# Zejun-Yang/AniPortrait

Measured on NVIDIA H100. Metric: denoised frames/sec @512x512 L=16 steps=25, higher is better.
Workload: dtype fp16

## Files before the change

### aniportrait_b200/csrc/ap_gemm.cu

```cuda
#include <stdio.h>
#include <stdlib.h>

#include "ap_host.h"
#include "ap_ptx.cuh"
#include "ap_wgmma.cuh"

namespace ap {

enum { A_GEMM = 0, A_CONV_S1 = 1, A_CONV_S2 = 2 };
enum { EPI_LINEAR = 0, EPI_GEGLU = 1 };

struct GemmParams {
  int M, N;
  int num_m_tiles, num_n_tiles, num_kb;
  int a_mode;
  int kb_src1, kb_src2;
  int Nf, Ho, Wo;
  int bw, bh, bn;
  int tiles_x, tiles_y;
  int C1, C2;
  const float* bias;
  int bias_group_rows;
  long long bias_ld;
  const __half* residual;
  int ldr;
  __half* out;
  int ldo;
  int out_al16, res_al16;
  int n_valid;
  int out_f32;
  int gelu;
  int quick_gelu;
  int tma_epi;
  int sub_w, sub_h, sub_n;
  int epi_double;
  int debug;
  float2* row_stat_out;
  long long row_stat_ld;
  float2* col_stat_out;
  long long col_stat_ld;
  const float* ln_rstd;
};


template <int BN, int EPI>
struct GemmCfg {
  static constexpr int BM = 128;
  static constexpr int BK = 64;
  static constexpr int A_BYTES = BM * BK * 2;
  static constexpr int B_BYTES = BN * BK * 2;
  static constexpr int STAGE_BYTES = A_BYTES + B_BYTES;
  static constexpr int EPI_STAGING = 8 * 4096;
  static constexpr int ACC_PW = EPI == EPI_GEGLU ? 128 : 64;
  static constexpr int ACC_LD = ACC_PW + 8;
  static constexpr int ACC_STAGING = 2 * 64 * ACC_LD * 4;
  static constexpr int MAX_SMEM = 227 * 1024 - 1024  - 256  - EPI_STAGING - ACC_STAGING;
  static constexpr int STAGES_RAW = MAX_SMEM / STAGE_BYTES;
  static constexpr int STAGES = STAGES_RAW > 8 ? 8 : STAGES_RAW;
  static constexpr int SMEM_BYTES = STAGES * STAGE_BYTES + EPI_STAGING + ACC_STAGING + 1024 + 256;
  static_assert(STAGES >= 2, "need at least a double-buffered operand ring");
  static_assert(B_BYTES % 1024 == 0, "B stage must keep 1024B alignment");
};


template <int BN, int EPI>
__global__ void __launch_bounds__(384, 1)
gemm_kernel(const __grid_constant__ CUtensorMap tmA1, const __grid_constant__ CUtensorMap tmA2,
            const __grid_constant__ CUtensorMap tmB, const __grid_constant__ CUtensorMap tmOut,
            const __grid_constant__ CUtensorMap tmRes, const GemmParams p) {
  using Cfg = GemmCfg<BN, EPI>;
  constexpr int STAGES = Cfg::STAGES;
  griddep_launch_dependents();
  extern __shared__ uint8_t smem_raw[];
  uint8_t* smem = reinterpret_cast<uint8_t*>((reinterpret_cast<uintptr_t>(smem_raw) + 1023) & ~uintptr_t(1023));
  uint8_t* smem_a = smem;
  uint8_t* smem_b = smem + STAGES * Cfg::A_BYTES;
  uint8_t* smem_epi = smem + STAGES * Cfg::STAGE_BYTES;
  float* smem_acc = reinterpret_cast<float*>(smem_epi + Cfg::EPI_STAGING);
  uint64_t* full_bar = reinterpret_cast<uint64_t*>(smem_acc + 2 * 64 * Cfg::ACC_LD);
  uint64_t* empty_bar = full_bar + STAGES;
  uint64_t* res_bar = empty_bar + STAGES;

  const int warp = threadIdx.x >> 5;
  const int lane = threadIdx.x & 31;
  const int n_groups = p.num_n_tiles;
  const int num_tiles = p.num_m_tiles * n_groups;
  const int first_tile = blockIdx.x;
  const int tile_stride = gridDim.x;

  if (warp == 0 && lane == 0) {
    tma_prefetch_desc(&tmA1);
    tma_prefetch_desc(&tmB);
    if (p.kb_src2 > 0) tma_prefetch_desc(&tmA2);
    for (int s = 0; s < STAGES; ++s) {
      mbar_init(&full_bar[s], 1);
      mbar_init(&empty_bar[s], 8);
    }
    for (int s = 0; s < 8; ++s) mbar_init(&res_bar[s], 1);
    if (p.tma_epi) {
      tma_prefetch_desc(&tmOut);
      if (p.residual != nullptr) tma_prefetch_desc(&tmRes);
    }
    fence_mbar_init();
  }
  __syncthreads();
  griddep_wait();

  if (warp < 4) {
    setmaxnreg_dec<40>();
    if (warp != 0) return;
    int stage = 0;
    uint32_t phase = 0;
    for (int tile = first_tile; tile < num_tiles; tile += tile_stride) {
      const int m_tile = tile / n_groups;
      const int n_tile = tile % n_groups;
      int n0 = 0, y0 = 0, x0 = 0;
      if (p.a_mode != A_GEMM) {
        const int per_frame = p.tiles_x * p.tiles_y;
        const int tn = m_tile / per_frame;
        const int rem = m_tile % per_frame;
        n0 = tn * p.bn;
        y0 = (rem / p.tiles_x) * p.bh;
        x0 = (rem % p.tiles_x) * p.bw;
      }
      int within = 0, kx = 0, ky = 0;
      for (int kb = 0; kb < p.num_kb; ++kb) {
        mbar_wait_quiet(&empty_bar[stage], phase ^ 1);
        if (elect_one()) {
          if (p.debug == 1) {
            mbar_arrive(&full_bar[stage]);
          } else {
            const bool load_a = !(p.debug == 4 && (kb & 1)), load_b = !(p.debug == 3 && (kb & 1));
            mbar_arrive_expect_tx(&full_bar[stage], (load_a ? Cfg::A_BYTES : 0) + (load_b ? Cfg::B_BYTES : 0));
            void* a_dst = smem_a + stage * Cfg::A_BYTES;
            void* b_dst = smem_b + stage * Cfg::B_BYTES;
            const bool second = within >= p.kb_src1;
            const CUtensorMap* am = second ? &tmA2 : &tmA1;
            const int c0 = (second ? within - p.kb_src1 : within) * Cfg::BK;
            if (!load_a) {
            } else if (p.a_mode == A_GEMM) {
              tma_load_2d(am, &full_bar[stage], a_dst, c0, m_tile * Cfg::BM);
            } else if (p.a_mode == A_CONV_S1) {
              tma_load_4d(am, &full_bar[stage], a_dst, c0, x0 + kx - 1, y0 + ky - 1, n0);
            } else {
              const int px = (kx == 1) ? 0 : 1, dx = (kx == 0) ? -1 : 0;
              const int py = (ky == 1) ? 0 : 1, dy = (ky == 0) ? -1 : 0;
              tma_load_5d(am, &full_bar[stage], a_dst, px * (second ? p.C2 : p.C1) + c0, x0 + dx, py, y0 + dy, n0);
            }
            if (load_b) tma_load_2d(&tmB, &full_bar[stage], b_dst, kb * Cfg::BK, n_tile * BN);
          }
        }
        __syncwarp();
        if (++within == p.kb_src1 + p.kb_src2) {
          within = 0;
          if (++kx == 3) { kx = 0; ++ky; }
        }
        if (++stage == STAGES) { stage = 0; phase ^= 1; }
      }
    }
    return;
  }

  setmaxnreg_inc<232>();
  const int wg = (warp >> 2) - 1;
  const int wq = warp & 3;
  const int lane_group = 2 * wg + (wq & 1);
  const int col_half = wq >> 1;
  const int row = lane_group * 32 + lane;
  const int r0 = lane_group * 32;
  float* acc_stage = smem_acc + wg * 64 * Cfg::ACC_LD;
  const float* acc_row = acc_stage + ((wq & 1) * 32 + lane) * Cfg::ACC_LD;
  constexpr int ACC_PER_CHUNK = (EPI == EPI_GEGLU) ? 64 : 32;
  constexpr int NCHUNK = BN / ACC_PER_CHUNK;
  constexpr int NPASS = (BN + Cfg::ACC_PW - 1) / Cfg::ACC_PW;
  const uint32_t a_base = smem_u32(smem_a) + wg * (64 * 128), b_base = smem_u32(smem_b);
  int stage = 0;
  uint32_t phase = 0;

  const int ew = warp - 4;
  uint8_t* obuf0 = smem_epi + ew * 4096;
  uint8_t* rbuf = obuf0 + 2048;
  uint32_t ochunk = 0;
  uint64_t* rbar = &res_bar[ew];
  uint32_t rphase = 0;
  const bool has_res = (EPI == EPI_LINEAR) && p.residual != nullptr;
  const int sw = (lane >> 1) & 3;
  float ln_next = 1.f;
  auto ln_prefetch = [&](int tile_) {
    if (tile_ >= num_tiles) return;
    const long long mm = (long long)(tile_ / n_groups) * Cfg::BM + r0 + lane;
    ln_next = mm < p.M ? __ldg(p.ln_rstd + mm) : 1.f;
  };
  if (p.tma_epi && p.ln_rstd != nullptr) ln_prefetch(first_tile);

  float acc[BN / 2];
  for (int tile = first_tile; tile < num_tiles; tile += tile_stride) {
    const int m_tile = tile / n_groups;
    const int n_tile = tile % n_groups;
    int prev_stage = -1;
    for (int kb = 0; kb < p.num_kb; ++kb) {
      mbar_wait_quiet(&full_bar[stage], phase);
      if (p.debug != 2) {
        wgmma_fence();
        const uint64_t da = wgmma_desc_k_sw128(a_base + stage * Cfg::A_BYTES);
        const uint64_t db = wgmma_desc_k_sw128(b_base + stage * Cfg::B_BYTES);
#pragma unroll
        for (int k = 0; k < Cfg::BK / 16; ++k) wgmma_ss<BN>(acc, da + 2 * k, db + 2 * k, (kb | k) != 0);
        wgmma_commit();
      }
      wgmma_wait<1>();
      if (prev_stage >= 0) {
        __syncwarp();
        if (lane == 0) mbar_arrive(&empty_bar[prev_stage]);
      }
      prev_stage = stage;
      if (++stage == STAGES) { stage = 0; phase ^= 1; }
    }
    wgmma_wait<0>();
    reg_fence<BN / 2>(acc);
    __syncwarp();
    if (lane == 0 && prev_stage >= 0) mbar_arrive(&empty_bar[prev_stage]);

    int cy = 0, cx = 0, cn = 0;
    long long m = 0;
    bool row_ok = true;
    if (p.a_mode == A_GEMM) {
      cy = m_tile * Cfg::BM + r0;
      m = (long long)cy + lane;
      row_ok = m < p.M;
    } else {
      const int per_frame = p.tiles_x * p.tiles_y;
      const int tn = m_tile / per_frame;
      const int rem = m_tile % per_frame;
      cn = tn * p.bn + r0 / (p.bh * p.bw);
      cy = (rem / p.tiles_x) * p.bh + (r0 / p.bw) % p.bh;
      cx = (rem % p.tiles_x) * p.bw + r0 % p.bw;
      const int n = tn * p.bn + row / (p.bh * p.bw);
      const int y = (rem / p.tiles_x) * p.bh + (row / p.bw) % p.bh;
      const int x = (rem % p.tiles_x) * p.bw + row % p.bw;
      row_ok = (n < p.Nf) && (y < p.Ho) && (x < p.Wo);
      m = ((long long)n * p.Ho + y) * p.Wo + x;
    }
    const float* bias_row = nullptr;
    if (p.bias != nullptr) bias_row = p.bias + (row_ok ? (m / p.bias_group_rows) : 0) * p.bias_ld;
    float ln_a = 1.f;
    if (p.tma_epi && p.ln_rstd != nullptr) {
      ln_a = ln_next;
      ln_prefetch(tile + tile_stride);
    }
    float rs_s = 0.f, rs_q = 0.f;
    const bool want_stats = (EPI == EPI_LINEAR) && (p.row_stat_out != nullptr || p.col_stat_out != nullptr);
    auto load_res = [&](int chunk) {
      if (lane == 0) {
        mbar_arrive_expect_tx(rbar, 2048);
        const int col = n_tile * BN + chunk * 32;
        if (p.a_mode == A_GEMM) tma_load_2d(&tmRes, rbar, rbuf, col, cy);
        else tma_load_4d(&tmRes, rbar, rbuf, col, cx, cy, cn);
      }
    };
    if (p.tma_epi && has_res && col_half < NCHUNK) load_res(col_half);

    auto chunk_tma = [&](int c, const float* src) {
      const int acol = n_tile * BN + c * ACC_PER_CHUNK;
      float v[32];
      if (EPI == EPI_GEGLU) {
#pragma unroll
        for (int h = 0; h < 2; ++h) {
          float bv[16], bg[16];
#pragma unroll
          for (int j = 0; j < 16; ++j) { bv[j] = 0.f; bg[j] = 0.f; }
          if (bias_row != nullptr) {
            const float4* b4 = reinterpret_cast<const float4*>(bias_row + acol + h * 32);
#pragma unroll
            for (int j = 0; j < 4; ++j) {
              const float4 a = __ldg(b4 + j), g = __ldg(b4 + 4 + j);
              bv[4 * j] = a.x; bv[4 * j + 1] = a.y; bv[4 * j + 2] = a.z; bv[4 * j + 3] = a.w;
              bg[4 * j] = g.x; bg[4 * j + 1] = g.y; bg[4 * j + 2] = g.z; bg[4 * j + 3] = g.w;
            }
          }
#pragma unroll
          for (int j = 0; j < 16; ++j)
            v[h * 16 + j] = fmaf(src[h * 32 + j], ln_a, bv[j]) * gelu_erf(fmaf(src[h * 32 + 16 + j], ln_a, bg[j]));
        }
      } else {
#pragma unroll
        for (int j = 0; j < 8; ++j) {
          const float4 a = reinterpret_cast<const float4*>(src)[j];
          v[4 * j] = a.x; v[4 * j + 1] = a.y; v[4 * j + 2] = a.z; v[4 * j + 3] = a.w;
        }
        if (p.ln_rstd != nullptr) {
          const float4* b4 = reinterpret_cast<const float4*>(bias_row + acol);
#pragma unroll
          for (int j = 0; j < 8; ++j) {
            const float4 b = __ldg(b4 + j);
            v[4 * j + 0] = fmaf(v[4 * j + 0], ln_a, b.x);
            v[4 * j + 1] = fmaf(v[4 * j + 1], ln_a, b.y);
            v[4 * j + 2] = fmaf(v[4 * j + 2], ln_a, b.z);
            v[4 * j + 3] = fmaf(v[4 * j + 3], ln_a, b.w);
          }
        } else if (bias_row != nullptr) {
          const float4* b4 = reinterpret_cast<const float4*>(bias_row + acol);
#pragma unroll
          for (int j = 0; j < 8; ++j) {
            const float4 b = __ldg(b4 + j);
            v[4 * j + 0] += b.x; v[4 * j + 1] += b.y; v[4 * j + 2] += b.z; v[4 * j + 3] += b.w;
          }
        }
        if (p.gelu) {
#pragma unroll
          for (int j = 0; j < 32; ++j) v[j] = gelu_erf(v[j]);
        } else if (p.quick_gelu) {
#pragma unroll
          for (int j = 0; j < 32; ++j) v[j] = quick_gelu(v[j]);
        }
        if (has_res) {
          mbar_wait_quiet(rbar, rphase);
          rphase ^= 1;
#pragma unroll
          for (int q = 0; q < 4; ++q) {
            const uint4 u = *reinterpret_cast<const uint4*>(rbuf + lane * 64 + ((q ^ sw) << 4));
            const __half2* h2 = reinterpret_cast<const __half2*>(&u);
#pragma unroll
            for (int j = 0; j < 4; ++j) {
              const float2 f = __half22float2(h2[j]);
              v[q * 8 + 2 * j] += f.x;
              v[q * 8 + 2 * j + 1] += f.y;
            }
          }
        }
      }
      const bool dbl = !has_res && p.epi_double;
      uint8_t* obuf = (dbl && (ochunk & 1)) ? rbuf : obuf0;
      ++ochunk;
      if (lane == 0) {
        if (dbl) tma_store_wait_read<1>();
        else tma_store_wait_read<0>();
      }
      __syncwarp();
      if (want_stats && !row_ok) {
#pragma unroll
        for (int j = 0; j < 32; ++j) v[j] = 0.f;
      }
#pragma unroll
      for (int q = 0; q < 4; ++q) {
        __half2 o[4];
#pragma unroll
        for (int j = 0; j < 4; ++j) o[j] = __floats2half2_rn(v[q * 8 + 2 * j], v[q * 8 + 2 * j + 1]);
        if (EPI == EPI_LINEAR && p.row_stat_out != nullptr) {
#pragma unroll
          for (int j = 0; j < 4; ++j) {
            const float2 f = __half22float2(o[j]);
            rs_s += f.x + f.y;
            rs_q = fmaf(f.x, f.x, fmaf(f.y, f.y, rs_q));
          }
        }
        *reinterpret_cast<uint4*>(obuf + lane * 64 + ((q ^ sw) << 4)) = *reinterpret_cast<uint4*>(o);
      }
      fence_proxy_async_smem();
      __syncwarp();
      if (EPI == EPI_LINEAR && p.col_stat_out != nullptr) {
        const int hc = lane & 15, rp = lane >> 4;
        float s0 = 0.f, s1 = 0.f, q0 = 0.f, q1 = 0.f;
#pragma unroll
        for (int rr = 0; rr < 16; ++rr) {
          const int rw = 2 * rr + rp;
          const uint32_t u = *reinterpret_cast<const uint32_t*>(
              obuf + rw * 64 + ((((hc >> 2) ^ ((rw >> 1) & 3))) << 4) + ((hc & 3) << 2));
          const float2 f = __half22float2(*reinterpret_cast<const __half2*>(&u));
          s0 += f.x; q0 = fmaf(f.x, f.x, q0);
          s1 += f.y; q1 = fmaf(f.y, f.y, q1);
        }
        s0 += __shfl_xor_sync(0xffffffffu, s0, 16);
        q0 += __shfl_xor_sync(0xffffffffu, q0, 16);
        s1 += __shfl_xor_sync(0xffffffffu, s1, 16);
        q1 += __shfl_xor_sync(0xffffffffu, q1, 16);
        if (lane < 16) {
          float4* dst = reinterpret_cast<float4*>(p.col_stat_out + (long long)(m_tile * 4 + lane_group) * p.col_stat_ld +
                                                  n_tile * BN + c * 32 + 2 * hc);
          *dst = make_float4(s0, q0, s1, q1);
        }
      }
      if (has_res && c + 2 < NCHUNK) load_res(c + 2);
      if (lane == 0) {
        const int ocol = n_tile * (BN / (EPI == EPI_GEGLU ? 2 : 1)) + c * 32;
        if (p.a_mode == A_GEMM) tma_store_2d(&tmOut, obuf, ocol, cy);
        else tma_store_4d(&tmOut, obuf, ocol, cx, cy, cn);
        tma_store_commit();
      }
    };

    auto chunk_direct = [&](int c, const float* src) {
      if (EPI == EPI_GEGLU) {
#pragma unroll
        for (int h = 0; h < 2; ++h) {
          const int ncol = n_tile * BN + c * 64 + h * 32;
          const float* s = src + h * 32;
          float v[32];
#pragma unroll
          for (int j = 0; j < 32; ++j) v[j] = s[j] + (bias_row != nullptr ? __ldg(bias_row + ncol + j) : 0.f);
          const int ocol = ncol >> 1;
          if (row_ok) {
            __half2 o[8];
#pragma unroll
            for (int j = 0; j < 8; ++j) {
              const float a0 = v[2 * j] * gelu_erf(v[16 + 2 * j]);
              const float a1 = v[2 * j + 1] * gelu_erf(v[16 + 2 * j + 1]);
              o[j] = __floats2half2_rn(a0, a1);
            }
            __half* dst = p.out + m * p.ldo + ocol;
            if (ocol + 16 <= p.n_valid && (p.ldo & 7) == 0 && p.out_al16) {
              uint4* d4 = reinterpret_cast<uint4*>(dst);
              d4[0] = *reinterpret_cast<uint4*>(&o[0]);
              d4[1] = *reinterpret_cast<uint4*>(&o[4]);
            } else {
              const __half* oh = reinterpret_cast<const __half*>(o);
              for (int j = 0; j < 16; ++j)
                if (ocol + j < p.n_valid) dst[j] = oh[j];
            }
          }
        }
        return;
      }
      const int ncol = n_tile * BN + c * 32;
      float v[32];
#pragma unroll
      for (int j = 0; j < 32; ++j) v[j] = src[j];
      if (bias_row != nullptr) {
        const float4* b4 = reinterpret_cast<const float4*>(bias_row + ncol);
#pragma unroll
        for (int j = 0; j < 8; ++j) {
          const float4 b = __ldg(b4 + j);
          v[4 * j + 0] += b.x; v[4 * j + 1] += b.y; v[4 * j + 2] += b.z; v[4 * j + 3] += b.w;
        }
      }
      if (p.gelu) {
#pragma unroll
        for (int j = 0; j < 32; ++j) v[j] = gelu_erf(v[j]);
      } else if (p.quick_gelu) {
#pragma unroll
        for (int j = 0; j < 32; ++j) v[j] = quick_gelu(v[j]);
      }
      if (!row_ok) return;
      const bool vec_ok = (ncol + 32 <= p.n_valid) && ((p.ldo & 7) == 0) && p.out_al16;
      if (p.residual != nullptr) {
        if (ncol + 32 <= p.n_valid && (p.ldr & 7) == 0 && p.res_al16) {
          const uint4* r4 = reinterpret_cast<const uint4*>(p.residual + m * p.ldr + ncol);
#pragma unroll
          for (int q = 0; q < 4; ++q) {
            const uint4 u = __ldg(r4 + q);
            const __half2* h2 = reinterpret_cast<const __half2*>(&u);
#pragma unroll
            for (int j = 0; j < 4; ++j) {
              const float2 f = __half22float2(h2[j]);
              v[q * 8 + 2 * j] += f.x;
              v[q * 8 + 2 * j + 1] += f.y;
            }
          }
        } else {
          const __half* rs = p.residual + m * p.ldr + ncol;
          for (int j = 0; j < 32; ++j)
            if (ncol + j < p.n_valid) v[j] += __half2float(rs[j]);
        }
      }
      __half* dst = p.out + m * p.ldo + ncol;
      if (p.out_f32) {
        float* dstf = reinterpret_cast<float*>(p.out) + m * p.ldo + ncol;
        for (int j = 0; j < 32; ++j)
          if (ncol + j < p.n_valid) dstf[j] = v[j];
      } else if (vec_ok) {
        uint4* d4 = reinterpret_cast<uint4*>(dst);
#pragma unroll
        for (int q = 0; q < 4; ++q) {
          __half2 o[4];
#pragma unroll
          for (int j = 0; j < 4; ++j) o[j] = __floats2half2_rn(v[q * 8 + 2 * j], v[q * 8 + 2 * j + 1]);
          d4[q] = *reinterpret_cast<uint4*>(o);
        }
      } else {
        for (int j = 0; j < 32; ++j)
          if (ncol + j < p.n_valid) dst[j] = __float2half_rn(v[j]);
      }
    };

#pragma unroll
    for (int ps = 0; ps < NPASS; ++ps) {
#pragma unroll
      for (int jl = 0; jl < Cfg::ACC_PW / 8; ++jl) {
        const int jn = ps * (Cfg::ACC_PW / 8) + jl;
        if (jn < BN / 8) {
          float* d0 = acc_stage + (wq * 16 + (lane >> 2)) * Cfg::ACC_LD + jl * 8 + 2 * (lane & 3);
          *reinterpret_cast<float2*>(d0) = make_float2(acc[4 * jn], acc[4 * jn + 1]);
          *reinterpret_cast<float2*>(d0 + 8 * Cfg::ACC_LD) = make_float2(acc[4 * jn + 2], acc[4 * jn + 3]);
        }
      }
      named_bar_sync(1 + wg, 128);
      const int c = ps * 2 + col_half;
      if (c < NCHUNK) {
        const float* src = acc_row + col_half * ACC_PER_CHUNK;
        if (p.tma_epi) chunk_tma(c, src);
        else chunk_direct(c, src);
      }
      named_bar_sync(1 + wg, 128);
    }
    if (p.tma_epi && EPI == EPI_LINEAR && p.row_stat_out != nullptr && row_ok)
      p.row_stat_out[(long long)(2 * n_tile + col_half) * p.row_stat_ld + m] = make_float2(rs_s, rs_q);
  }
  if (p.tma_epi && lane == 0) tma_store_wait_all<0>();
}

template <int BN, int EPI>
static int launch_gemm(const CUtensorMap& a1, const CUtensorMap& a2, const CUtensorMap& b, const CUtensorMap& to,
                       const CUtensorMap& tr, const GemmParams& p, cudaStream_t stream) {
  using Cfg = GemmCfg<BN, EPI>;
  static bool attr_set = false;
  if (!attr_set) {
    AP_CHECK_CUDA(cudaFuncSetAttribute(gemm_kernel<BN, EPI>, cudaFuncAttributeMaxDynamicSharedMemorySize,
                                       Cfg::SMEM_BYTES));
    attr_set = true;
  }
  const int items = p.num_m_tiles * p.num_n_tiles;
  const int grid = items < num_sms() ? items : num_sms();
  {
    cudaError_t le = launch_pdl(gemm_kernel<BN, EPI>, dim3(grid), dim3(384), (size_t)Cfg::SMEM_BYTES, stream, 1, a1, a2,
                                b, to, tr, p);
    if (le != cudaSuccess) return fail(AP_ERR_CUDA, "gemm launch: %s", cudaGetErrorString(le));
  }
  AP_CHECK_CUDA(cudaGetLastError());
  return AP_OK;
}

static int pick_bn(int N, int forced, long long m_tiles, bool geglu = false) {
  if (forced > 0) return forced;
  const int cand[4] = {160, 128, 64, 32};
  const double quality[4] = {0.95, 0.90, 0.70, 0.45};
  int best = -1;
  double best_score = -1.0;
  const int sms = num_sms();
  for (int i = 0; i < 4; ++i) {
    if (N % cand[i] != 0) continue;
    if (geglu && cand[i] % 64 != 0) continue;
    const long long tiles = m_tiles * (N / cand[i]);
    const long long waves = (tiles + sms - 1) / sms;
    const double fill = (double)tiles / (double)(waves * sms);
    const double score = fill * quality[i];
    if (score > best_score + 1e-9) { best_score = score; best = cand[i]; }
  }
  return best;
}

static int dispatch(int bn, int epi, const CUtensorMap& a1, const CUtensorMap& a2, const CUtensorMap& b,
                    const CUtensorMap& to, const CUtensorMap& tr, const GemmParams& p, cudaStream_t stream) {
  if (epi == EPI_GEGLU) {
    switch (bn) {
      case 128: return launch_gemm<128, EPI_GEGLU>(a1, a2, b, to, tr, p, stream);
      case 64: return launch_gemm<64, EPI_GEGLU>(a1, a2, b, to, tr, p, stream);
      default: return fail(AP_ERR_INVALID, "gemm: unsupported GEGLU BLOCK_N %d", bn);
    }
  }
  switch (bn) {
    case 256: return launch_gemm<256, EPI_LINEAR>(a1, a2, b, to, tr, p, stream);
    case 160: return launch_gemm<160, EPI_LINEAR>(a1, a2, b, to, tr, p, stream);
    case 128: return launch_gemm<128, EPI_LINEAR>(a1, a2, b, to, tr, p, stream);
    case 64: return launch_gemm<64, EPI_LINEAR>(a1, a2, b, to, tr, p, stream);
    case 32: return launch_gemm<32, EPI_LINEAR>(a1, a2, b, to, tr, p, stream);
    default: return fail(AP_ERR_INVALID, "gemm: unsupported BLOCK_N %d", bn);
  }
}

static int make_weight_map(CUtensorMap* tm, const void* w, int N, long long K, int bn_box) {
  const uint64_t dims[2] = {(uint64_t)K, (uint64_t)N};
  const uint64_t strides[1] = {(uint64_t)K * 2};
  const uint32_t box[2] = {64, (uint32_t)bn_box};
  return encode_tmap(tm, w, 2, dims, strides, box, true);
}

static int apply_ext(GemmParams& p, const ap_epilogue_ext* ext, int epi, long long m_pad, int k_ln) {
  p.bias_ld = p.N;
  static const int epi_double = getenv("AP_GEMM_EPI_DOUBLE") ? atoi(getenv("AP_GEMM_EPI_DOUBLE")) : 1;
  p.epi_double = epi_double;
  if (ext != nullptr && ext->bias_ld > 0) p.bias_ld = ext->bias_ld;
  if (p.bias != nullptr && ((reinterpret_cast<uintptr_t>(p.bias) & 15) != 0 || (p.bias_ld & 3) != 0))
    return fail(AP_ERR_INVALID, "gemm: bias must be 16-byte aligned with bias_ld %% 4 == 0 (bias_ld %lld)", p.bias_ld);
  if (ext == nullptr) return AP_OK;
  const bool any = ext->row_stat_out || ext->col_stat_out || ext->ln_rstd;
  if (!any) return AP_OK;
  if (!p.tma_epi) return fail(AP_ERR_INVALID, "gemm: epilogue statistics / LayerNorm folding need the TMA epilogue (aligned fp16 out)");
  if ((ext->row_stat_out || ext->col_stat_out) && p.n_valid < (epi == EPI_GEGLU ? p.N / 2 : p.N))
    return fail(AP_ERR_INVALID, "gemm: row / column statistics need n_valid (%d) == the output width", p.n_valid);
  if (ext->row_stat_out) {
    if (epi != EPI_LINEAR) return fail(AP_ERR_INVALID, "gemm: row statistics are not available with GEGLU");
    if (ext->row_stat_ld < m_pad) return fail(AP_ERR_INVALID, "gemm: row_stat_ld %lld < padded M %lld", ext->row_stat_ld, m_pad);
    if (p.a_mode != A_GEMM) return fail(AP_ERR_INVALID, "gemm: row statistics only for plain GEMMs");
    p.row_stat_out = (float2*)ext->row_stat_out;
    p.row_stat_ld = ext->row_stat_ld;
  }
  if (ext->col_stat_out) {
    if (epi != EPI_LINEAR) return fail(AP_ERR_INVALID, "gemm: column statistics are not available with GEGLU");
    if (ext->col_stat_ld < p.N || (ext->col_stat_ld & 1)) return fail(AP_ERR_INVALID, "gemm: bad col_stat_ld %lld", ext->col_stat_ld);
    if ((reinterpret_cast<uintptr_t>(ext->col_stat_out) & 15) != 0) return fail(AP_ERR_INVALID, "gemm: col_stat_out must be 16-byte aligned");
    if (p.a_mode != A_GEMM && p.sub_n != 1)
      return fail(AP_ERR_INVALID, "conv3x3: column statistics need Ho*Wo %% 32 == 0 with 32-row sub-boxes inside one frame");
    p.col_stat_out = (float2*)ext->col_stat_out;
    p.col_stat_ld = ext->col_stat_ld;
  }
  if (ext->ln_rstd) {
    if (p.a_mode != A_GEMM) return fail(AP_ERR_INVALID, "gemm: LayerNorm folding only for plain GEMMs");
    if (p.bias == nullptr) return fail(AP_ERR_INVALID, "gemm: LayerNorm folding needs the folded bias (beta.W^T + b)");
    p.ln_rstd = ext->ln_rstd;
  }
  return AP_OK;
}

}

using namespace ap;

extern "C" int ap_gemm_row_stat_parts(long long M, int N, int K, int flags, int block_n) {
// ... 184 lines not shown
```

Before: 5.677.

## Add dedicated epilogue warps with smem accumulator handoff for GEGLU and short-K GEMMs

Adds a GEMM kernel variant with separate epilogue warps (one or two extra warpgroups). The math warpgroups dump their accumulators into a full 128xBN shared-memory tile and signal an mbarrier, so the epilogue of one tile can overlap the MMA main loop of the next. The old kernel is kept as the fused variant, and the handoff variant is chosen only for GEGLU and for BN=160 GEMMs with few K blocks. The residual and output staging buffers are also reworked to double-buffer residual loads and allow up to four in-flight TMA stores. In exchange, the full accumulator staging uses more shared memory, which leaves fewer pipeline stages. The setmaxnreg rebalancing is also dropped in the new kernel, which may leave the MMA warps short of registers.

```diff
diff --git a/aniportrait_b200/csrc/ap_gemm.cu b/aniportrait_b200/csrc/ap_gemm.cu
--- a/aniportrait_b200/csrc/ap_gemm.cu
+++ b/aniportrait_b200/csrc/ap_gemm.cu
@@ -1,5 +1,7 @@
 #include <stdio.h>
 #include <stdlib.h>
+
+#include <type_traits>
 
 #include "ap_host.h"
 #include "ap_ptx.cuh"
@@ -50,10 +52,12 @@
   static constexpr int A_BYTES = BM * BK * 2;
   static constexpr int B_BYTES = BN * BK * 2;
   static constexpr int STAGE_BYTES = A_BYTES + B_BYTES;
-  static constexpr int EPI_STAGING = 8 * 4096;
-  static constexpr int ACC_PW = EPI == EPI_GEGLU ? 128 : 64;
-  static constexpr int ACC_LD = ACC_PW + 8;
-  static constexpr int ACC_STAGING = 2 * 64 * ACC_LD * 4;
+  static constexpr int NEPI = EPI == EPI_GEGLU ? 2 : 1;
+  static constexpr int THREADS = 384 + 128 * NEPI;
+  static constexpr int EPI_WARP_BYTES = EPI == EPI_GEGLU ? 2048 : 8192;
+  static constexpr int EPI_STAGING = 4 * NEPI * EPI_WARP_BYTES;
+  static constexpr int ACC_LD = BN + 8;
+  static constexpr int ACC_STAGING = BM * ACC_LD * 4;
   static constexpr int MAX_SMEM = 227 * 1024 - 1024  - 256  - EPI_STAGING - ACC_STAGING;
   static constexpr int STAGES_RAW = MAX_SMEM / STAGE_BYTES;
   static constexpr int STAGES = STAGES_RAW > 8 ? 8 : STAGES_RAW;
@@ -64,7 +68,7 @@
 
 
 template <int BN, int EPI>
-__global__ void __launch_bounds__(384, 1)
+__global__ void __launch_bounds__(GemmCfg<BN, EPI>::THREADS, 1)
 gemm_kernel(const __grid_constant__ CUtensorMap tmA1, const __grid_constant__ CUtensorMap tmA2,
             const __grid_constant__ CUtensorMap tmB, const __grid_constant__ CUtensorMap tmOut,
             const __grid_constant__ CUtensorMap tmRes, const GemmParams p) {
@@ -77,9 +81,11 @@
   uint8_t* smem_b = smem + STAGES * Cfg::A_BYTES;
   uint8_t* smem_epi = smem + STAGES * Cfg::STAGE_BYTES;
   float* smem_acc = reinterpret_cast<float*>(smem_epi + Cfg::EPI_STAGING);
-  uint64_t* full_bar = reinterpret_cast<uint64_t*>(smem_acc + 2 * 64 * Cfg::ACC_LD);
+  uint64_t* full_bar = reinterpret_cast<uint64_t*>(smem_acc + Cfg::BM * Cfg::ACC_LD);
   uint64_t* empty_bar = full_bar + STAGES;
   uint64_t* res_bar = empty_bar + STAGES;
+  uint64_t* acc_full = res_bar + 8;
+  uint64_t* acc_empty = acc_full + 1;
 
   const int warp = threadIdx.x >> 5;
   const int lane = threadIdx.x & 31;
@@ -97,6 +103,8 @@
       mbar_init(&empty_bar[s], 8);
     }
     for (int s = 0; s < 8; ++s) mbar_init(&res_bar[s], 1);
+    mbar_init(acc_full, 256);
+    mbar_init(acc_empty, 128 * Cfg::NEPI);
     if (p.tma_epi) {
       tma_prefetch_desc(&tmOut);
       if (p.residual != nullptr) tma_prefetch_desc(&tmRes);
@@ -107,7 +115,6 @@
   griddep_wait();
 
   if (warp < 4) {
-    setmaxnreg_dec<40>();
     if (warp != 0) return;
     int stage = 0;
     uint32_t phase = 0;
@@ -161,29 +168,65 @@
     return;
   }
 
-  setmaxnreg_inc<232>();
-  const int wg = (warp >> 2) - 1;
-  const int wq = warp & 3;
-  const int lane_group = 2 * wg + (wq & 1);
-  const int col_half = wq >> 1;
-  const int row = lane_group * 32 + lane;
-  const int r0 = lane_group * 32;
-  float* acc_stage = smem_acc + wg * 64 * Cfg::ACC_LD;
-  const float* acc_row = acc_stage + ((wq & 1) * 32 + lane) * Cfg::ACC_LD;
+  if (warp < 12) {
+    const int wg = (warp >> 2) - 1;
+    const int wq = warp & 3;
+    const uint32_t a_base = smem_u32(smem_a) + wg * (64 * 128), b_base = smem_u32(smem_b);
+    int stage = 0;
+    uint32_t phase = 0, acc_phase = 0;
+    float acc[BN / 2];
+    for (int tile = first_tile; tile < num_tiles; tile += tile_stride) {
+      int prev_stage = -1;
+      for (int kb = 0; kb < p.num_kb; ++kb) {
+        mbar_wait_quiet(&full_bar[stage], phase);
+        if (p.debug != 2) {
+          wgmma_fence();
+          const uint64_t da = wgmma_desc_k_sw128(a_base + stage * Cfg::A_BYTES);
+          const uint64_t db = wgmma_desc_k_sw128(b_base + stage * Cfg::B_BYTES);
+#pragma unroll
+          for (int k = 0; k < Cfg::BK / 16; ++k) wgmma_ss<BN>(acc, da + 2 * k, db + 2 * k, (kb | k) != 0);
+          wgmma_commit();
+        }
+        wgmma_wait<1>();
+        if (prev_stage >= 0) {
+          __syncwarp();
+          if (lane == 0) mbar_arrive(&empty_bar[prev_stage]);
+        }
+        prev_stage = stage;
+        if (++stage == STAGES) { stage = 0; phase ^= 1; }
+      }
+      wgmma_wait<0>();
+      reg_fence<BN / 2>(acc);
+      __syncwarp();
+      if (lane == 0 && prev_stage >= 0) mbar_arrive(&empty_bar[prev_stage]);
+      mbar_wait_quiet(acc_empty, acc_phase ^ 1);
+#pragma unroll
+      for (int jn = 0; jn < BN / 8; ++jn) {
+        float* d0 = smem_acc + (wg * 64 + wq * 16 + (lane >> 2)) * Cfg::ACC_LD + jn * 8 + 2 * (lane & 3);
+        *reinterpret_cast<float2*>(d0) = make_float2(acc[4 * jn], acc[4 * jn + 1]);
+        *reinterpret_cast<float2*>(d0 + 8 * Cfg::ACC_LD) = make_float2(acc[4 * jn + 2], acc[4 * jn + 3]);
+      }
+      mbar_arrive(acc_full);
+      acc_phase ^= 1;
+    }
+    return;
+  }
+
+  const int ew = warp - 12;
+  const int rq = ew & 3;
+  const int cp = ew >> 2;
+  const int row = rq * 32 + lane;
+  const int r0 = rq * 32;
+  const float* acc_row = smem_acc + row * Cfg::ACC_LD;
   constexpr int ACC_PER_CHUNK = (EPI == EPI_GEGLU) ? 64 : 32;
   constexpr int NCHUNK = BN / ACC_PER_CHUNK;
-  constexpr int NPASS = (BN + Cfg::ACC_PW - 1) / Cfg::ACC_PW;
-  const uint32_t a_base = smem_u32(smem_a) + wg * (64 * 128), b_base = smem_u32(smem_b);
-  int stage = 0;
-  uint32_t phase = 0;
-
-  const int ew = warp - 4;
-  uint8_t* obuf0 = smem_epi + ew * 4096;
-  uint8_t* rbuf = obuf0 + 2048;
+  uint32_t acc_phase = 0;
+
+  uint8_t* wbuf = smem_epi + ew * Cfg::EPI_WARP_BYTES;
+  const bool has_res = (EPI == EPI_LINEAR) && p.residual != nullptr;
+  const int nout = (EPI == EPI_GEGLU || !p.epi_double) ? 1 : (has_res ? 2 : 4);
   uint32_t ochunk = 0;
-  uint64_t* rbar = &res_bar[ew];
   uint32_t rphase = 0;
-  const bool has_res = (EPI == EPI_LINEAR) && p.residual != nullptr;
   const int sw = (lane >> 1) & 3;
   float ln_next = 1.f;
   auto ln_prefetch = [&](int tile_) {
@@ -193,34 +236,9 @@
   };
   if (p.tma_epi && p.ln_rstd != nullptr) ln_prefetch(first_tile);
 
-  float acc[BN / 2];
   for (int tile = first_tile; tile < num_tiles; tile += tile_stride) {
     const int m_tile = tile / n_groups;
     const int n_tile = tile % n_groups;
-    int prev_stage = -1;
-    for (int kb = 0; kb < p.num_kb; ++kb) {
-      mbar_wait_quiet(&full_bar[stage], phase);
-      if (p.debug != 2) {
-        wgmma_fence();
-        const uint64_t da = wgmma_desc_k_sw128(a_base + stage * Cfg::A_BYTES);
-        const uint64_t db = wgmma_desc_k_sw128(b_base + stage * Cfg::B_BYTES);
-#pragma unroll
-        for (int k = 0; k < Cfg::BK / 16; ++k) wgmma_ss<BN>(acc, da + 2 * k, db + 2 * k, (kb | k) != 0);
-        wgmma_commit();
-      }
-      wgmma_wait<1>();
-      if (prev_stage >= 0) {
-        __syncwarp();
-        if (lane == 0) mbar_arrive(&empty_bar[prev_stage]);
-      }
-      prev_stage = stage;
-      if (++stage == STAGES) { stage = 0; phase ^= 1; }
-    }
-    wgmma_wait<0>();
-    reg_fence<BN / 2>(acc);
-    __syncwarp();
-    if (lane == 0 && prev_stage >= 0) mbar_arrive(&empty_bar[prev_stage]);
-
     int cy = 0, cx = 0, cn = 0;
     long long m = 0;
     bool row_ok = true;
@@ -248,17 +266,22 @@
       ln_a = ln_next;
       ln_prefetch(tile + tile_stride);
     }
-    float rs_s = 0.f, rs_q = 0.f;
+    float rs_s0 = 0.f, rs_q0 = 0.f, rs_s1 = 0.f, rs_q1 = 0.f;
     const bool want_stats = (EPI == EPI_LINEAR) && (p.row_stat_out != nullptr || p.col_stat_out != nullptr);
     auto load_res = [&](int chunk) {
       if (lane == 0) {
+        uint64_t* rbar = &res_bar[2 * ew + (chunk & 1)];
+        uint8_t* rbuf = wbuf + (2 + (chunk & 1)) * 2048;
         mbar_arrive_expect_tx(rbar, 2048);
         const int col = n_tile * BN + chunk * 32;
         if (p.a_mode == A_GEMM) tma_load_2d(&tmRes, rbar, rbuf, col, cy);
         else tma_load_4d(&tmRes, rbar, rbuf, col, cx, cy, cn);
       }
     };
-    if (p.tma_epi && has_res && col_half < NCHUNK) load_res(col_half);
+    if (p.tma_epi && has_res) {
+      load_res(0);
+      if (NCHUNK > 1) load_res(1);
+    }
 
     auto chunk_tma = [&](int c, const float* src) {
       const int acol = n_tile * BN + c * ACC_PER_CHUNK;
@@ -314,8 +337,9 @@
           for (int j = 0; j < 32; ++j) v[j] = quick_gelu(v[j]);
         }
         if (has_res) {
-          mbar_wait_quiet(rbar, rphase);
-          rphase ^= 1;
+          const uint8_t* rbuf = wbuf + (2 + (c & 1)) * 2048;
+          mbar_wait_quiet(&res_bar[2 * ew + (c & 1)], (rphase >> (c & 1)) & 1);
+          rphase ^= 1u << (c & 1);
 #pragma unroll
           for (int q = 0; q < 4; ++q) {
             const uint4 u = *reinterpret_cast<const uint4*>(rbuf + lane * 64 + ((q ^ sw) << 4));
@@ -327,13 +351,15 @@
               v[q * 8 + 2 * j + 1] += f.y;
             }
           }
-        }
-      }
-      const bool dbl = !has_res && p.epi_double;
-      uint8_t* obuf = (dbl && (ochunk & 1)) ? rbuf : obuf0;
+          __syncwarp();
+          if (c + 2 < NCHUNK) load_res(c + 2);
+        }
+      }
+      uint8_t* obuf = wbuf + (ochunk % nout) * 2048;
       ++ochunk;
       if (lane == 0) {
-        if (dbl) tma_store_wait_read<1>();
+        if (nout == 4) tma_store_wait_read<3>();
+        else if (nout == 2) tma_store_wait_read<1>();
         else tma_store_wait_read<0>();
       }
       __syncwarp();
@@ -341,6 +367,7 @@
 #pragma unroll
         for (int j = 0; j < 32; ++j) v[j] = 0.f;
       }
+      float rs_s = (c & 1) ? rs_s1 : rs_s0, rs_q = (c & 1) ? rs_q1 : rs_q0;
 #pragma unroll
       for (int q = 0; q < 4; ++q) {
         __half2 o[4];
@@ -356,6 +383,7 @@
         }
         *reinterpret_cast<uint4*>(obuf + lane * 64 + ((q ^ sw) << 4)) = *reinterpret_cast<uint4*>(o);
       }
+      if (c & 1) { rs_s1 = rs_s; rs_q1 = rs_q; } else { rs_s0 = rs_s; rs_q0 = rs_q; }
       fence_proxy_async_smem();
       __syncwarp();
       if (EPI == EPI_LINEAR && p.col_stat_out != nullptr) {
@@ -375,12 +403,11 @@
         s1 += __shfl_xor_sync(0xffffffffu, s1, 16);
         q1 += __shfl_xor_sync(0xffffffffu, q1, 16);
         if (lane < 16) {
-          float4* dst = reinterpret_cast<float4*>(p.col_stat_out + (long long)(m_tile * 4 + lane_group) * p.col_stat_ld +
+          float4* dst = reinterpret_cast<float4*>(p.col_stat_out + (long long)(m_tile * 4 + rq) * p.col_stat_ld +
                                                   n_tile * BN + c * 32 + 2 * hc);
           *dst = make_float4(s0, q0, s1, q1);
         }
       }
-      if (has_res && c + 2 < NCHUNK) load_res(c + 2);
       if (lane == 0) {
         const int ocol = n_tile * (BN / (EPI == EPI_GEGLU ? 2 : 1)) + c * 32;
         if (p.a_mode == A_GEMM) tma_store_2d(&tmOut, obuf, ocol, cy);
@@ -482,6 +509,461 @@
       }
     };
 
+    mbar_wait_quiet(acc_full, acc_phase);
+    for (int c = cp; c < NCHUNK; c += Cfg::NEPI) {
+      if (p.tma_epi) chunk_tma(c, acc_row + c * ACC_PER_CHUNK);
+      else chunk_direct(c, acc_row + c * ACC_PER_CHUNK);
+    }
+    mbar_arrive(acc_empty);
+    acc_phase ^= 1;
+    if (p.tma_epi && EPI == EPI_LINEAR && p.row_stat_out != nullptr && row_ok) {
+      p.row_stat_out[(long long)(2 * n_tile) * p.row_stat_ld + m] = make_float2(rs_s0, rs_q0);
+      p.row_stat_out[(long long)(2 * n_tile + 1) * p.row_stat_ld + m] = make_float2(rs_s1, rs_q1);
+    }
+  }
+  if (p.tma_epi && lane == 0) tma_store_wait_all<0>();
+}
+
+template <int BN, int EPI>
+struct FusedGemmCfg {
+  static constexpr int THREADS = 384;
+  static constexpr int BM = 128;
+  static constexpr int BK = 64;
+  static constexpr int A_BYTES = BM * BK * 2;
+  static constexpr int B_BYTES = BN * BK * 2;
+  static constexpr int STAGE_BYTES = A_BYTES + B_BYTES;
+  static constexpr int EPI_STAGING = 8 * 4096;
+  static constexpr int ACC_PW = EPI == EPI_GEGLU ? 128 : 64;
+  static constexpr int ACC_LD = ACC_PW + 8;
+  static constexpr int ACC_STAGING = 2 * 64 * ACC_LD * 4;
+  static constexpr int MAX_SMEM = 227 * 1024 - 1024  - 256  - EPI_STAGING - ACC_STAGING;
+  static constexpr int STAGES_RAW = MAX_SMEM / STAGE_BYTES;
+  static constexpr int STAGES = STAGES_RAW > 8 ? 8 : STAGES_RAW;
+  static constexpr int SMEM_BYTES = STAGES * STAGE_BYTES + EPI_STAGING + ACC_STAGING + 1024 + 256;
+  static_assert(STAGES >= 2, "need at least a double-buffered operand ring");
+  static_assert(B_BYTES % 1024 == 0, "B stage must keep 1024B alignment");
+};
+
+
+template <int BN, int EPI>
+__global__ void __launch_bounds__(384, 1)
+gemm_fused_kernel(const __grid_constant__ CUtensorMap tmA1, const __grid_constant__ CUtensorMap tmA2,
+            const __grid_constant__ CUtensorMap tmB, const __grid_constant__ CUtensorMap tmOut,
+            const __grid_constant__ CUtensorMap tmRes, const GemmParams p) {
+  using Cfg = FusedGemmCfg<BN, EPI>;
+  constexpr int STAGES = Cfg::STAGES;
+  griddep_launch_dependents();
+  extern __shared__ uint8_t smem_raw[];
+  uint8_t* smem = reinterpret_cast<uint8_t*>((reinterpret_cast<uintptr_t>(smem_raw) + 1023) & ~uintptr_t(1023));
+  uint8_t* smem_a = smem;
+  uint8_t* smem_b = smem + STAGES * Cfg::A_BYTES;
+  uint8_t* smem_epi = smem + STAGES * Cfg::STAGE_BYTES;
+  float* smem_acc = reinterpret_cast<float*>(smem_epi + Cfg::EPI_STAGING);
+  uint64_t* full_bar = reinterpret_cast<uint64_t*>(smem_acc + 2 * 64 * Cfg::ACC_LD);
+  uint64_t* empty_bar = full_bar + STAGES;
+  uint64_t* res_bar = empty_bar + STAGES;
+
+  const int warp = threadIdx.x >> 5;
+  const int lane = threadIdx.x & 31;
+  const int n_groups = p.num_n_tiles;
+  const int num_tiles = p.num_m_tiles * n_groups;
+  const int first_tile = blockIdx.x;
+  const int tile_stride = gridDim.x;
+
+  if (warp == 0 && lane == 0) {
+    tma_prefetch_desc(&tmA1);
+    tma_prefetch_desc(&tmB);
+    if (p.kb_src2 > 0) tma_prefetch_desc(&tmA2);
+    for (int s = 0; s < STAGES; ++s) {
+      mbar_init(&full_bar[s], 1);
+      mbar_init(&empty_bar[s], 8);
+    }
+    for (int s = 0; s < 8; ++s) mbar_init(&res_bar[s], 1);
+    if (p.tma_epi) {
+      tma_prefetch_desc(&tmOut);
+      if (p.residual != nullptr) tma_prefetch_desc(&tmRes);
+    }
+    fence_mbar_init();
+  }
+  __syncthreads();
+  griddep_wait();
+
+  if (warp < 4) {
+    setmaxnreg_dec<40>();
+    if (warp != 0) return;
+    int stage = 0;
+    uint32_t phase = 0;
+    for (int tile = first_tile; tile < num_tiles; tile += tile_stride) {
+      const int m_tile = tile / n_groups;
+      const int n_tile = tile % n_groups;
+      int n0 = 0, y0 = 0, x0 = 0;
+      if (p.a_mode != A_GEMM) {
+        const int per_frame = p.tiles_x * p.tiles_y;
+        const int tn = m_tile / per_frame;
+        const int rem = m_tile % per_frame;
+        n0 = tn * p.bn;
+        y0 = (rem / p.tiles_x) * p.bh;
+        x0 = (rem % p.tiles_x) * p.bw;
+      }
+      int within = 0, kx = 0, ky = 0;
+      for (int kb = 0; kb < p.num_kb; ++kb) {
+        mbar_wait_quiet(&empty_bar[stage], phase ^ 1);
+        if (elect_one()) {
+          if (p.debug == 1) {
+            mbar_arrive(&full_bar[stage]);
+          } else {
+            const bool load_a = !(p.debug == 4 && (kb & 1)), load_b = !(p.debug == 3 && (kb & 1));
+            mbar_arrive_expect_tx(&full_bar[stage], (load_a ? Cfg::A_BYTES : 0) + (load_b ? Cfg::B_BYTES : 0));
+            void* a_dst = smem_a + stage * Cfg::A_BYTES;
+            void* b_dst = smem_b + stage * Cfg::B_BYTES;
+            const bool second = within >= p.kb_src1;
+            const CUtensorMap* am = second ? &tmA2 : &tmA1;
+            const int c0 = (second ? within - p.kb_src1 : within) * Cfg::BK;
+            if (!load_a) {
+            } else if (p.a_mode == A_GEMM) {
+              tma_load_2d(am, &full_bar[stage], a_dst, c0, m_tile * Cfg::BM);
+            } else if (p.a_mode == A_CONV_S1) {
+              tma_load_4d(am, &full_bar[stage], a_dst, c0, x0 + kx - 1, y0 + ky - 1, n0);
+            } else {
+              const int px = (kx == 1) ? 0 : 1, dx = (kx == 0) ? -1 : 0;
+              const int py = (ky == 1) ? 0 : 1, dy = (ky == 0) ? -1 : 0;
+              tma_load_5d(am, &full_bar[stage], a_dst, px * (second ? p.C2 : p.C1) + c0, x0 + dx, py, y0 + dy, n0);
+            }
+            if (load_b) tma_load_2d(&tmB, &full_bar[stage], b_dst, kb * Cfg::BK, n_tile * BN);
+          }
+        }
+        __syncwarp();
+        if (++within == p.kb_src1 + p.kb_src2) {
+          within = 0;
+          if (++kx == 3) { kx = 0; ++ky; }
+        }
+        if (++stage == STAGES) { stage = 0; phase ^= 1; }
+      }
+    }
+    return;
+  }
+
+  setmaxnreg_inc<232>();
+  const int wg = (warp >> 2) - 1;
+  const int wq = warp & 3;
+  const int lane_group = 2 * wg + (wq & 1);
+  const int col_half = wq >> 1;
+  const int row = lane_group * 32 + lane;
+  const int r0 = lane_group * 32;
+  float* acc_stage = smem_acc + wg * 64 * Cfg::ACC_LD;
+  const float* acc_row = acc_stage + ((wq & 1) * 32 + lane) * Cfg::ACC_LD;
+  constexpr int ACC_PER_CHUNK = (EPI == EPI_GEGLU) ? 64 : 32;
+  constexpr int NCHUNK = BN / ACC_PER_CHUNK;
+  constexpr int NPASS = (BN + Cfg::ACC_PW - 1) / Cfg::ACC_PW;
+  const uint32_t a_base = smem_u32(smem_a) + wg * (64 * 128), b_base = smem_u32(smem_b);
+  int stage = 0;
+  uint32_t phase = 0;
+
+  const int ew = warp - 4;
+  uint8_t* obuf0 = smem_epi + ew * 4096;
+  uint8_t* rbuf = obuf0 + 2048;
+  uint32_t ochunk = 0;
+  uint64_t* rbar = &res_bar[ew];
+  uint32_t rphase = 0;
+  const bool has_res = (EPI == EPI_LINEAR) && p.residual != nullptr;
+  const int sw = (lane >> 1) & 3;
+  float ln_next = 1.f;
+  auto ln_prefetch = [&](int tile_) {
+    if (tile_ >= num_tiles) return;
+    const long long mm = (long long)(tile_ / n_groups) * Cfg::BM + r0 + lane;
+    ln_next = mm < p.M ? __ldg(p.ln_rstd + mm) : 1.f;
+  };
+  if (p.tma_epi && p.ln_rstd != nullptr) ln_prefetch(first_tile);
+
+  float acc[BN / 2];
+  for (int tile = first_tile; tile < num_tiles; tile += tile_stride) {
+    const int m_tile = tile / n_groups;
+    const int n_tile = tile % n_groups;
+    int prev_stage = -1;
+    for (int kb = 0; kb < p.num_kb; ++kb) {
+      mbar_wait_quiet(&full_bar[stage], phase);
+      if (p.debug != 2) {
+        wgmma_fence();
+        const uint64_t da = wgmma_desc_k_sw128(a_base + stage * Cfg::A_BYTES);
+        const uint64_t db = wgmma_desc_k_sw128(b_base + stage * Cfg::B_BYTES);
+#pragma unroll
+        for (int k = 0; k < Cfg::BK / 16; ++k) wgmma_ss<BN>(acc, da + 2 * k, db + 2 * k, (kb | k) != 0);
+        wgmma_commit();
+      }
+      wgmma_wait<1>();
+      if (prev_stage >= 0) {
+        __syncwarp();
+        if (lane == 0) mbar_arrive(&empty_bar[prev_stage]);
+      }
+      prev_stage = stage;
+      if (++stage == STAGES) { stage = 0; phase ^= 1; }
+    }
+    wgmma_wait<0>();
+    reg_fence<BN / 2>(acc);
+    __syncwarp();
+    if (lane == 0 && prev_stage >= 0) mbar_arrive(&empty_bar[prev_stage]);
+
+    int cy = 0, cx = 0, cn = 0;
+    long long m = 0;
+    bool row_ok = true;
+    if (p.a_mode == A_GEMM) {
+      cy = m_tile * Cfg::BM + r0;
+      m = (long long)cy + lane;
+      row_ok = m < p.M;
+    } else {
+      const int per_frame = p.tiles_x * p.tiles_y;
+      const int tn = m_tile / per_frame;
+      const int rem = m_tile % per_frame;
+      cn = tn * p.bn + r0 / (p.bh * p.bw);
+      cy = (rem / p.tiles_x) * p.bh + (r0 / p.bw) % p.bh;
+      cx = (rem % p.tiles_x) * p.bw + r0 % p.bw;
+      const int n = tn * p.bn + row / (p.bh * p.bw);
+      const int y = (rem / p.tiles_x) * p.bh + (row / p.bw) % p.bh;
+      const int x = (rem % p.tiles_x) * p.bw + row % p.bw;
+      row_ok = (n < p.Nf) && (y < p.Ho) && (x < p.Wo);
+      m = ((long long)n * p.Ho + y) * p.Wo + x;
+    }
+    const float* bias_row = nullptr;
+    if (p.bias != nullptr) bias_row = p.bias + (row_ok ? (m / p.bias_group_rows) : 0) * p.bias_ld;
+    float ln_a = 1.f;
+    if (p.tma_epi && p.ln_rstd != nullptr) {
+      ln_a = ln_next;
+      ln_prefetch(tile + tile_stride);
+    }
+    float rs_s = 0.f, rs_q = 0.f;
+    const bool want_stats = (EPI == EPI_LINEAR) && (p.row_stat_out != nullptr || p.col_stat_out != nullptr);
+    auto load_res = [&](int chunk) {
+      if (lane == 0) {
+        mbar_arrive_expect_tx(rbar, 2048);
+        const int col = n_tile * BN + chunk * 32;
+        if (p.a_mode == A_GEMM) tma_load_2d(&tmRes, rbar, rbuf, col, cy);
+        else tma_load_4d(&tmRes, rbar, rbuf, col, cx, cy, cn);
+      }
+    };
+    if (p.tma_epi && has_res && col_half < NCHUNK) load_res(col_half);
+
+    auto chunk_tma = [&](int c, const float* src) {
+      const int acol = n_tile * BN + c * ACC_PER_CHUNK;
+      float v[32];
+      if (EPI == EPI_GEGLU) {
+#pragma unroll
+        for (int h = 0; h < 2; ++h) {
+          float bv[16], bg[16];
+#pragma unroll
+          for (int j = 0; j < 16; ++j) { bv[j] = 0.f; bg[j] = 0.f; }
+          if (bias_row != nullptr) {
+            const float4* b4 = reinterpret_cast<const float4*>(bias_row + acol + h * 32);
+#pragma unroll
+            for (int j = 0; j < 4; ++j) {
+              const float4 a = __ldg(b4 + j), g = __ldg(b4 + 4 + j);
+              bv[4 * j] = a.x; bv[4 * j + 1] = a.y; bv[4 * j + 2] = a.z; bv[4 * j + 3] = a.w;
+              bg[4 * j] = g.x; bg[4 * j + 1] = g.y; bg[4 * j + 2] = g.z; bg[4 * j + 3] = g.w;
+            }
+          }
+#pragma unroll
+          for (int j = 0; j < 16; ++j)
+            v[h * 16 + j] = fmaf(src[h * 32 + j], ln_a, bv[j]) * gelu_erf(fmaf(src[h * 32 + 16 + j], ln_a, bg[j]));
+        }
+      } else {
+#pragma unroll
+        for (int j = 0; j < 8; ++j) {
+          const float4 a = reinterpret_cast<const float4*>(src)[j];
+          v[4 * j] = a.x; v[4 * j + 1] = a.y; v[4 * j + 2] = a.z; v[4 * j + 3] = a.w;
+        }
+        if (p.ln_rstd != nullptr) {
+          const float4* b4 = reinterpret_cast<const float4*>(bias_row + acol);
+#pragma unroll
+          for (int j = 0; j < 8; ++j) {
+            const float4 b = __ldg(b4 + j);
+            v[4 * j + 0] = fmaf(v[4 * j + 0], ln_a, b.x);
+            v[4 * j + 1] = fmaf(v[4 * j + 1], ln_a, b.y);
+            v[4 * j + 2] = fmaf(v[4 * j + 2], ln_a, b.z);
+            v[4 * j + 3] = fmaf(v[4 * j + 3], ln_a, b.w);
+          }
+        } else if (bias_row != nullptr) {
+          const float4* b4 = reinterpret_cast<const float4*>(bias_row + acol);
+#pragma unroll
+          for (int j = 0; j < 8; ++j) {
+            const float4 b = __ldg(b4 + j);
+            v[4 * j + 0] += b.x; v[4 * j + 1] += b.y; v[4 * j + 2] += b.z; v[4 * j + 3] += b.w;
+          }
+        }
+        if (p.gelu) {
+#pragma unroll
+          for (int j = 0; j < 32; ++j) v[j] = gelu_erf(v[j]);
+        } else if (p.quick_gelu) {
+#pragma unroll
+          for (int j = 0; j < 32; ++j) v[j] = quick_gelu(v[j]);
+        }
+        if (has_res) {
+          mbar_wait_quiet(rbar, rphase);
+          rphase ^= 1;
+#pragma unroll
+          for (int q = 0; q < 4; ++q) {
+            const uint4 u = *reinterpret_cast<const uint4*>(rbuf + lane * 64 + ((q ^ sw) << 4));
+            const __half2* h2 = reinterpret_cast<const __half2*>(&u);
+#pragma unroll
+            for (int j = 0; j < 4; ++j) {
+              const float2 f = __half22float2(h2[j]);
+              v[q * 8 + 2 * j] += f.x;
+              v[q * 8 + 2 * j + 1] += f.y;
+            }
+          }
+        }
+      }
+      const bool dbl = !has_res && p.epi_double;
+      uint8_t* obuf = (dbl && (ochunk & 1)) ? rbuf : obuf0;
+      ++ochunk;
+      if (lane == 0) {
+        if (dbl) tma_store_wait_read<1>();
+        else tma_store_wait_read<0>();
+      }
+      __syncwarp();
+      if (want_stats && !row_ok) {
+#pragma unroll
+        for (int j = 0; j < 32; ++j) v[j] = 0.f;
+      }
+#pragma unroll
+      for (int q = 0; q < 4; ++q) {
+        __half2 o[4];
+#pragma unroll
+        for (int j = 0; j < 4; ++j) o[j] = __floats2half2_rn(v[q * 8 + 2 * j], v[q * 8 + 2 * j + 1]);
+        if (EPI == EPI_LINEAR && p.row_stat_out != nullptr) {
+#pragma unroll
+          for (int j = 0; j < 4; ++j) {
+            const float2 f = __half22float2(o[j]);
+            rs_s += f.x + f.y;
+            rs_q = fmaf(f.x, f.x, fmaf(f.y, f.y, rs_q));
+          }
+        }
+        *reinterpret_cast<uint4*>(obuf + lane * 64 + ((q ^ sw) << 4)) = *reinterpret_cast<uint4*>(o);
+      }
+      fence_proxy_async_smem();
+      __syncwarp();
+      if (EPI == EPI_LINEAR && p.col_stat_out != nullptr) {
+        const int hc = lane & 15, rp = lane >> 4;
+        float s0 = 0.f, s1 = 0.f, q0 = 0.f, q1 = 0.f;
+#pragma unroll
+        for (int rr = 0; rr < 16; ++rr) {
+          const int rw = 2 * rr + rp;
+          const uint32_t u = *reinterpret_cast<const uint32_t*>(
+              obuf + rw * 64 + ((((hc >> 2) ^ ((rw >> 1) & 3))) << 4) + ((hc & 3) << 2));
+          const float2 f = __half22float2(*reinterpret_cast<const __half2*>(&u));
+          s0 += f.x; q0 = fmaf(f.x, f.x, q0);
+          s1 += f.y; q1 = fmaf(f.y, f.y, q1);
+        }
+        s0 += __shfl_xor_sync(0xffffffffu, s0, 16);
+        q0 += __shfl_xor_sync(0xffffffffu, q0, 16);
+        s1 += __shfl_xor_sync(0xffffffffu, s1, 16);
+        q1 += __shfl_xor_sync(0xffffffffu, q1, 16);
+        if (lane < 16) {
+          float4* dst = reinterpret_cast<float4*>(p.col_stat_out + (long long)(m_tile * 4 + lane_group) * p.col_stat_ld +
+                                                  n_tile * BN + c * 32 + 2 * hc);
+          *dst = make_float4(s0, q0, s1, q1);
+        }
+      }
+      if (has_res && c + 2 < NCHUNK) load_res(c + 2);
+      if (lane == 0) {
+        const int ocol = n_tile * (BN / (EPI == EPI_GEGLU ? 2 : 1)) + c * 32;
+        if (p.a_mode == A_GEMM) tma_store_2d(&tmOut, obuf, ocol, cy);
+        else tma_store_4d(&tmOut, obuf, ocol, cx, cy, cn);
+        tma_store_commit();
+      }
+    };
+
+    auto chunk_direct = [&](int c, const float* src) {
+      if (EPI == EPI_GEGLU) {
+#pragma unroll
+        for (int h = 0; h < 2; ++h) {
+          const int ncol = n_tile * BN + c * 64 + h * 32;
+          const float* s = src + h * 32;
+          float v[32];
+#pragma unroll
+          for (int j = 0; j < 32; ++j) v[j] = s[j] + (bias_row != nullptr ? __ldg(bias_row + ncol + j) : 0.f);
+          const int ocol = ncol >> 1;
+          if (row_ok) {
+            __half2 o[8];
+#pragma unroll
+            for (int j = 0; j < 8; ++j) {
+              const float a0 = v[2 * j] * gelu_erf(v[16 + 2 * j]);
+              const float a1 = v[2 * j + 1] * gelu_erf(v[16 + 2 * j + 1]);
+              o[j] = __floats2half2_rn(a0, a1);
+            }
+            __half* dst = p.out + m * p.ldo + ocol;
+            if (ocol + 16 <= p.n_valid && (p.ldo & 7) == 0 && p.out_al16) {
+              uint4* d4 = reinterpret_cast<uint4*>(dst);
+              d4[0] = *reinterpret_cast<uint4*>(&o[0]);
+              d4[1] = *reinterpret_cast<uint4*>(&o[4]);
+            } else {
+              const __half* oh = reinterpret_cast<const __half*>(o);
+              for (int j = 0; j < 16; ++j)
+                if (ocol + j < p.n_valid) dst[j] = oh[j];
+            }
+          }
+        }
+        return;
+      }
+      const int ncol = n_tile * BN + c * 32;
+      float v[32];
+#pragma unroll
+      for (int j = 0; j < 32; ++j) v[j] = src[j];
+      if (bias_row != nullptr) {
+        const float4* b4 = reinterpret_cast<const float4*>(bias_row + ncol);
+#pragma unroll
+        for (int j = 0; j < 8; ++j) {
+          const float4 b = __ldg(b4 + j);
+          v[4 * j + 0] += b.x; v[4 * j + 1] += b.y; v[4 * j + 2] += b.z; v[4 * j + 3] += b.w;
+        }
+      }
+      if (p.gelu) {
+#pragma unroll
+        for (int j = 0; j < 32; ++j) v[j] = gelu_erf(v[j]);
+      } else if (p.quick_gelu) {
+#pragma unroll
+        for (int j = 0; j < 32; ++j) v[j] = quick_gelu(v[j]);
+      }
+      if (!row_ok) return;
+      const bool vec_ok = (ncol + 32 <= p.n_valid) && ((p.ldo & 7) == 0) && p.out_al16;
+      if (p.residual != nullptr) {
+        if (ncol + 32 <= p.n_valid && (p.ldr & 7) == 0 && p.res_al16) {
+          const uint4* r4 = reinterpret_cast<const uint4*>(p.residual + m * p.ldr + ncol);
+#pragma unroll
+          for (int q = 0; q < 4; ++q) {
+            const uint4 u = __ldg(r4 + q);
+            const __half2* h2 = reinterpret_cast<const __half2*>(&u);
+#pragma unroll
+            for (int j = 0; j < 4; ++j) {
+              const float2 f = __half22float2(h2[j]);
+              v[q * 8 + 2 * j] += f.x;
+              v[q * 8 + 2 * j + 1] += f.y;
+            }
+          }
+        } else {
+          const __half* rs = p.residual + m * p.ldr + ncol;
+          for (int j = 0; j < 32; ++j)
+            if (ncol + j < p.n_valid) v[j] += __half2float(rs[j]);
+        }
+      }
+      __half* dst = p.out + m * p.ldo + ncol;
+      if (p.out_f32) {
+        float* dstf = reinterpret_cast<float*>(p.out) + m * p.ldo + ncol;
+        for (int j = 0; j < 32; ++j)
+          if (ncol + j < p.n_valid) dstf[j] = v[j];
+      } else if (vec_ok) {
+        uint4* d4 = reinterpret_cast<uint4*>(dst);
+#pragma unroll
+        for (int q = 0; q < 4; ++q) {
+          __half2 o[4];
+#pragma unroll
+          for (int j = 0; j < 4; ++j) o[j] = __floats2half2_rn(v[q * 8 + 2 * j], v[q * 8 + 2 * j + 1]);
+          d4[q] = *reinterpret_cast<uint4*>(o);
+        }
+      } else {
+        for (int j = 0; j < 32; ++j)
+          if (ncol + j < p.n_valid) dst[j] = __float2half_rn(v[j]);
+      }
+    };
+
 #pragma unroll
     for (int ps = 0; ps < NPASS; ++ps) {
 #pragma unroll
@@ -508,25 +990,33 @@
   if (p.tma_epi && lane == 0) tma_store_wait_all<0>();
 }
 
-template <int BN, int EPI>
+template <int BN, int EPI, bool HANDOFF>
 static int launch_gemm(const CUtensorMap& a1, const CUtensorMap& a2, const CUtensorMap& b, const CUtensorMap& to,
                        const CUtensorMap& tr, const GemmParams& p, cudaStream_t stream) {
-  using Cfg = GemmCfg<BN, EPI>;
+  using Cfg = typename std::conditional<HANDOFF, GemmCfg<BN, EPI>, FusedGemmCfg<BN, EPI>>::type;
+  const auto kernel = [] {
+    if constexpr (HANDOFF) return gemm_kernel<BN, EPI>;
+    else return gemm_fused_kernel<BN, EPI>;
+  }();
   static bool attr_set = false;
   if (!attr_set) {
-    AP_CHECK_CUDA(cudaFuncSetAttribute(gemm_kernel<BN, EPI>, cudaFuncAttributeMaxDynamicSharedMemorySize,
-                                       Cfg::SMEM_BYTES));
+    AP_CHECK_CUDA(cudaFuncSetAttribute(kernel, cudaFuncAttributeMaxDynamicSharedMemorySize, Cfg::SMEM_BYTES));
     attr_set = true;
   }
   const int items = p.num_m_tiles * p.num_n_tiles;
   const int grid = items < num_sms() ? items : num_sms();
   {
-    cudaError_t le = launch_pdl(gemm_kernel<BN, EPI>, dim3(grid), dim3(384), (size_t)Cfg::SMEM_BYTES, stream, 1, a1, a2,
+    cudaError_t le = launch_pdl(kernel, dim3(grid), dim3(Cfg::THREADS), (size_t)Cfg::SMEM_BYTES, stream, 1, a1, a2,
                                 b, to, tr, p);
     if (le != cudaSuccess) return fail(AP_ERR_CUDA, "gemm launch: %s", cudaGetErrorString(le));
   }
   AP_CHECK_CUDA(cudaGetLastError());
   return AP_OK;
+}
+
+static bool use_handoff(int bn, int epi, const GemmParams& p) {
+  if (p.a_mode != A_GEMM) return false;
+  return epi == EPI_GEGLU || (bn == 160 && p.num_kb <= 10);
 }
 
 static int pick_bn(int N, int forced, long long m_tiles, bool geglu = false) {
@@ -550,19 +1040,23 @@
 
 static int dispatch(int bn, int epi, const CUtensorMap& a1, const CUtensorMap& a2, const CUtensorMap& b,
                     const CUtensorMap& to, const CUtensorMap& tr, const GemmParams& p, cudaStream_t stream) {
+  const bool h = use_handoff(bn, epi, p);
   if (epi == EPI_GEGLU) {
     switch (bn) {
-      case 128: return launch_gemm<128, EPI_GEGLU>(a1, a2, b, to, tr, p, stream);
-      case 64: return launch_gemm<64, EPI_GEGLU>(a1, a2, b, to, tr, p, stream);
+      case 128: return h ? launch_gemm<128, EPI_GEGLU, true>(a1, a2, b, to, tr, p, stream)
+                         : launch_gemm<128, EPI_GEGLU, false>(a1, a2, b, to, tr, p, stream);
+      case 64: return h ? launch_gemm<64, EPI_GEGLU, true>(a1, a2, b, to, tr, p, stream)
+                        : launch_gemm<64, EPI_GEGLU, false>(a1, a2, b, to, tr, p, stream);
       default: return fail(AP_ERR_INVALID, "gemm: unsupported GEGLU BLOCK_N %d", bn);
     }
   }
   switch (bn) {
-    case 256: return launch_gemm<256, EPI_LINEAR>(a1, a2, b, to, tr, p, stream);
-    case 160: return launch_gemm<160, EPI_LINEAR>(a1, a2, b, to, tr, p, stream);
-    case 128: return launch_gemm<128, EPI_LINEAR>(a1, a2, b, to, tr, p, stream);
-    case 64: return launch_gemm<64, EPI_LINEAR>(a1, a2, b, to, tr, p, stream);
-    case 32: return launch_gemm<32, EPI_LINEAR>(a1, a2, b, to, tr, p, stream);
+    case 256: return launch_gemm<256, EPI_LINEAR, false>(a1, a2, b, to, tr, p, stream);
+    case 160: return h ? launch_gemm<160, EPI_LINEAR, true>(a1, a2, b, to, tr, p, stream)
+                       : launch_gemm<160, EPI_LINEAR, false>(a1, a2, b, to, tr, p, stream);
+    case 128: return launch_gemm<128, EPI_LINEAR, false>(a1, a2, b, to, tr, p, stream);
+    case 64: return launch_gemm<64, EPI_LINEAR, false>(a1, a2, b, to, tr, p, stream);
+    case 32: return launch_gemm<32, EPI_LINEAR, false>(a1, a2, b, to, tr, p, stream);
     default: return fail(AP_ERR_INVALID, "gemm: unsupported BLOCK_N %d", bn);
   }
 }
```

Result: faster. 5.742, median of 6 (+1.1%).
